# google-research/rigl

Measured on AMD Instinct MI355X. Metric: images/sec/node, ResNet-50 80% ERK RigL step, higher is better.
Workload: dtype bf16

## Files before the change

### rigl_amd/csrc/conv.hip

```cpp
#include <stdlib.h>

#include "common.hpp"

#if defined(RIGL_ABLATE) && RIGL_ABLATE == 1
#define RIGL_MFMA_OR_ABLATE(i, j) acc[i][j][0] += (float)af[i][0] + (float)bfr[j][0];
#else
#define RIGL_MFMA_OR_ABLATE(i, j) acc[i][j] = __builtin_amdgcn_mfma_f32_32x32x16_bf16(bfr[j], af[i], acc[i][j], 0, 0, 0);
#endif

namespace rigl {
namespace k1 {

typedef __attribute__((ext_vector_type(8))) __bf16 bf16x8;
typedef __attribute__((ext_vector_type(2))) __bf16 bf16x2;
typedef __attribute__((ext_vector_type(2))) float f32x2;
typedef __attribute__((ext_vector_type(16))) float f32x16;

constexpr int THREADS = 256;

__device__ __forceinline__ uint16_t f2bf(float f) {
  uint32_t u = __float_as_uint(f);
  if ((u & 0x7FFFFFFFu) > 0x7F800000u) return (uint16_t)((u >> 16) | 0x40u);
  u += 0x7FFFu + ((u >> 16) & 1u);
  return (uint16_t)(u >> 16);
// ... 1089 lines not shown
  return pl;
}

template <int MODE, bool F32>
static void launch_igemm(const IgemmArgs& a0, hipStream_t st) {
  IgemmArgs a = a0;
  const IgemmPlan pl = plan_igemm<MODE>(a);
  if (!F32 && pl.big) {
    RIGL_K_LAUNCH((k_igemm_big<MODE, false>), dim3(pl.grid), dim3(512), (igemm_smem_bytes<2, 2, 32, MODE, false, false, 3, 4>()), st, a);
    return;
  }
  if (pl.cls) launch_igemm_t<MODE, F32, true>(a, dim3(pl.grid), pl.wide_n, pl.dma, st);
  else launch_igemm_t<MODE, F32, false>(a, dim3(pl.grid), pl.wide_n, pl.dma, st);
}

static int check_desc(const RiglConvDesc* d, const char* who) {
  if (!d) return fail(RIGL_EINVAL, "%s: NULL descriptor", who);
  if (d->n <= 0 || d->h <= 0 || d->w <= 0 || d->cin <= 0 || d->ho <= 0 || d->wo <= 0 || d->cout <= 0 || d->kh <= 0 ||
      d->kw <= 0 || d->stride_h <= 0 || d->stride_w <= 0 || d->pad_top < 0 || d->pad_left < 0)
    return fail(RIGL_EINVAL, "%s: non-positive dimension in descriptor", who);
  if ((d->ho - 1) * d->stride_h - d->pad_top >= d->h || (d->wo - 1) * d->stride_w - d->pad_left >= d->w)
    return fail(RIGL_EINVAL, "%s: output size inconsistent with input/stride/pad", who);
  const int64_t lim = (int64_t(1) << 30) - 1;
  if ((int64_t)d->n * d->h * d->w * d->cin > lim || (int64_t)d->n * d->ho * d->wo * d->cout > lim ||
      (int64_t)d->kh * d->kw * d->cin * d->cout > lim)
    return fail(RIGL_EUNSUPPORTED, "%s: tensor exceeds 2^30 elements", who);
  return RIGL_OK;
}

static inline bool small_cin(const RiglConvDesc* d) { return (d->cin % 8) != 0 && d->cin > 4; }
static inline int kpad(const RiglConvDesc* d) { return (d->kh * d->kw * d->cin + 31) / 32 * 32; }

#include "convpp.hpp"
#include "bwd1x1.hpp"
#include "stem.hpp"
#include "c3x3.hpp"
#include "rowstream.hpp"
#include "bwdslice.hpp"

static size_t pp_ksplit_workspace(const RiglConvDesc* d) {
  if (d->cin <= 4 || (d->cin % 8) || (d->cout % 8)) return 0;
  IgemmArgs a = {};
  a.M = d->n * d->ho * d->wo; a.N = d->cout; a.Cred = d->cin; a.a_pix_stride = d->cin; a.KH = d->kh; a.KW = d->kw;
  a.RH = d->ho; a.RW = d->wo; a.GH = d->h; a.GW = d->w; a.sh = d->stride_h; a.sw = d->stride_w;
  const PPPlan p = plan_pp<0>(a);
  if (!pp_ksplit_ok(a, p)) return 0;
  return (size_t)p.grid * 2 * p.bm * p.bn * 4 + align_up((size_t)p.grid * 4, 256);
}

struct WgradPlan { int tm, tn, tiles_ci, tiles_co, splits; int64_t slab; };
static int wgrad_stages(int tm, int tn) { return (tm == 2 && tn == 2) ? 3 : 4; }
static int num_cus() {
  static const int n = [] {
    int dev = 0, v = 0;
    if (hipGetDevice(&dev) != hipSuccess || hipDeviceGetAttribute(&v, hipDeviceAttributeMultiprocessorCount, dev) != hipSuccess || v <= 0) v = 256;
    return v;
  }();
  return n;
}
static WgradPlan plan_wgrad(int M, int cin, int cout, int taps, bool fused = false) {
  WgradPlan p;
  p.tm = cin > 64 ? 2 : 1;
  p.tn = cout > 64 ? 2 : 1;
  p.tiles_ci = (cin + 64 * p.tm - 1) / (64 * p.tm);
  p.tiles_co = (cout + 64 * p.tn - 1) / (64 * p.tn);
  const int64_t base = (int64_t)p.tiles_ci * p.tiles_co * taps;
  const int kt = (M + 63) / 64;
  const int target = 0;
  const int lds = wgrad_stages(p.tm, p.tn) * 32 * 64 * (p.tm + p.tn) * 2;
  const int lds_cu = 160 * 1024;
  int occ = lds_cu / lds;
  if (occ > 4) occ = 4;
  int64_t slots = target > 0 ? target : (int64_t)num_cus() * occ;
  static const int fused_pct = [] { const char* e = getenv("RIGL_WGRAD_FUSED_PCT"); return e ? atoi(e) : 60; }();
  static const int fused_pct_small = [] { const char* e = getenv("RIGL_WGRAD_FUSED_PCT_SMALL"); return e ? atoi(e) : 75; }();
  if (fused && target <= 0) slots = slots * ((p.tm == 2 && p.tn == 2) ? fused_pct : fused_pct_small) / 100;
  int64_t s = slots / base;
  if (s > kt / 4) s = kt / 4;
  if (s < 1) s = 1;
  if (s > 1024) s = 1024;
  p.splits = (int)s;
  p.slab = (int64_t)taps * cin * cout;
  return p;
}

static WgradPlan tiny_wgrad_plan(int M, int cred, int cout, int kh) { return plan_wgrad(M, kh * cred, cout, 1); }

}
}

extern "C" {

size_t rigl_conv2d_workspace_bytes(const RiglConvDesc* d, int32_t which) {
  using namespace rigl;
  using namespace rigl::k1;
  if (!d) return 0;
  const int64_t M = (int64_t)d->n * d->ho * d->wo;
  if (tiny_cin(d)) {
    const TinyGeom tg = tiny_geom(d);
    const size_t xp = align_up((size_t)d->n * tg.hp * tg.wp * 4 * 2, 256);
    if (which == 0) return xp + align_up((size_t)d->cout * d->kh * tg.cred * 2, 256);
    if (which == 2) {
      WgradPlan p = tiny_wgrad_plan((int)M, tg.cred, d->cout, d->kh);
      const size_t generic = xp + align_up((size_t)p.slab * 4, 256) + align_up((size_t)p.splits * p.slab * 4, 256);
      const size_t direct = stem_wgrad_workspace(d);
      return generic > direct ? generic : direct;
    }
    return 0;
  }
  if (small_cin(d)) {
    const int Kp = kpad(d);
    size_t col = align_up((size_t)M * Kp * 2, 256);
    if (which == 0) return col + align_up((size_t)d->cout * Kp * 2, 256);
    if (which == 2) {
      WgradPlan p = plan_wgrad((int)M, Kp, d->cout, 1);
      return col + align_up((size_t)p.splits * p.slab * 4, 256);
    }
    return 0;
  }
  if (which == 0) return pp_ksplit_workspace(d);
  if (which == 2) {
    WgradPlan p = plan_wgrad((int)M, d->cin, d->cout, d->kh * d->kw);
    size_t need = p.splits > 1 ? align_up((size_t)p.splits * p.slab * 4, 256) : 0;
    const size_t npp = align_up(pp_wgrad_workspace(d), 256);
    if (npp > need) need = npp;
    const size_t n11 = align_up(bwd1x1_workspace(d), 256);
    if (n11 > need) need = n11;
    const size_t n33 = align_up(c3x3_wgrad_workspace(d), 256);
    if (n33 > need) need = n33;
    const size_t nbs = align_up(bs_workspace(d), 256);
    if (nbs > need) need = nbs;
    return need;
  }
  return 0;
}

int32_t rigl_conv2d_stats_parts(const RiglConvDesc* d) {
  if (!d || d->cout <= 0 || (d->cout % 8)) return 0;
  const int64_t M = (int64_t)d->n * d->ho * d->wo;
  using namespace rigl::k1;
  if (c3x3_use(d)) return c3x3_stats_parts(d);
  { RsPlan rp; if (rs_use<0>(d, &rp)) return rp.gprime; }
  return (int32_t)((M + 127) / 128);
}

int rigl_masked_conv2d_fwd_stats(const RiglConvDesc* d, const rigl_bf16* x, const rigl_bf16* w_ohwi, rigl_bf16* y,
                                 float* stats, size_t stats_floats, void* workspace, size_t workspace_bytes,
                                 rigl_stream_t stream) {
  using namespace rigl;
  using namespace rigl::k1;
  int rc = check_desc(d, "rigl_masked_conv2d_fwd");
  if (rc) return rc;
  if (!x || !w_ohwi || !y) return fail(RIGL_EINVAL, "rigl_masked_conv2d_fwd: NULL tensor");
  if (d->cout % 8) return fail(RIGL_EUNSUPPORTED, "rigl_masked_conv2d_fwd: cout %% 8 != 0 (use the reference kernel)");
  if (stats && stats_floats < (size_t)rigl_conv2d_stats_parts(d) * 2 * d->cout)
    return fail(RIGL_EWORKSPACE, "rigl_masked_conv2d_fwd_stats: stats buffer %zu floats < %zu", stats_floats,
                (size_t)rigl_conv2d_stats_parts(d) * 2 * d->cout);
  hipStream_t st = as_stream(stream);
  prof_set_tag(d);
  ProfFamily prof(PROF_CONV_FWD);
  IgemmArgs a = {};
  a.C = y; a.M = d->n * d->ho * d->wo; a.N = d->cout; a.ldc = d->cout; a.STATS = stats;
  const size_t need = rigl_conv2d_workspace_bytes(d, 0);
  if ((tiny_cin(d) || small_cin(d)) && need && (!workspace || workspace_bytes < need))
    return fail(RIGL_EWORKSPACE, "rigl_masked_conv2d_fwd: workspace %zu < %zu", workspace_bytes, need);
  if (tiny_cin(d)) {
// ... 563 lines not shown
```

### rigl_amd/csrc/convpp.hpp

```cpp
#pragma once

template <int WM, int WN, int TM, int TN, int PH>
struct PPGeom {
  static_assert(PH == 2 || PH == 1, "phases per K-tile");
  static constexpr int NST = PH == 1 ? 3 : 2;
  static_assert(WM * WN == 8, "eight waves");
  static_assert(TM % 2 == 0 && TN % 2 == 0, "a wave tile splits into 2 x 2 quadrants");
  static constexpr int BM = WM * TM * 32, BN = WN * TN * 32;
  static constexpr int AH_ROWS = BM / 2, BH_ROWS = BN / 2;
  static constexpr int AH_BYTES = AH_ROWS * 128, BH_BYTES = BH_ROWS * 128;
  static constexpr int STAGE = 2 * AH_BYTES + 2 * BH_BYTES;
  static constexpr int NA = AH_ROWS / 64, NB = BH_ROWS / 64;
  static_assert(AH_ROWS % 64 == 0 && BH_ROWS % 64 == 0, "a piece is whole rounds of 8 waves x 8 rows");
  static constexpr int QM = TM / 2, QN = TN / 2;
  static constexpr int EPI_ROWB = TN * 64 + 16;
  static constexpr int EPI_WAVE = QM * 32 * EPI_ROWB;
  static constexpr int EPI_STATS = 8 * EPI_WAVE;
  static constexpr int EPI_ALL = EPI_STATS + 8 * 2 * TN * 32 * 4;
  static constexpr int SMEM = (NST * STAGE > EPI_ALL) ? NST * STAGE : EPI_ALL;
  static_assert(SMEM <= 160 * 1024, "LDS per CU");
};

#define PP_BARRIER()                                                                                     \
  {                                                                                                      \
// ... 242 lines not shown
          const f32x16& a = acc[h * QM + i][j];
          const f32x2 lo = {a[4 * q], a[4 * q + 1]}, hi2 = {a[4 * q + 2], a[4 * q + 3]};
          uint2 pk;
          pk.x = __builtin_bit_cast(uint32_t, __builtin_convertvector(lo, bf16x2));
          pk.y = __builtin_bit_cast(uint32_t, __builtin_convertvector(hi2, bf16x2));
          *reinterpret_cast<uint2*>(stg + row * ROWB + col * 2) = pk;
        }
    const int mrow0 = m0 + wm * TM * 32 + h * QM * 32;
    int mout[ITERS];
#pragma unroll
    for (int it = 0; it < ITERS; ++it) {
      const int lm = mrow0 + it * RPI + rsub;
      if (CLS) {
        int n, rh, rw;
        const int mm = lm < c_cnt ? lm : 0;
        PP_ROW_PIXEL(mm, n, rh, rw);
        mout[it] = lm < c_cnt ? (n * P.RH + rh) * P.RW + rw : -1;
      } else {
        mout[it] = lm < P.M ? lm : -1;
      }
    }
    uint4 addv[ITERS];
    if (P.ADD) {
#pragma unroll
      for (int it = 0; it < ITERS; ++it)
        addv[it] = mout[it] >= 0 ? *reinterpret_cast<const uint4*>(P.ADD + (int64_t)mout[it] * P.ldc + ncol) : make_uint4(0u, 0u, 0u, 0u);
    }
#pragma unroll
    for (int it = 0; it < ITERS; ++it) {
      const int row = it * RPI + rsub, m = mout[it];
      uint4 v = *reinterpret_cast<const uint4*>(stg + row * ROWB + ch * 16);
      if (MODE == 0 && P.STATS) {
        const uint32_t vw[4] = {v.x, v.y, v.z, v.w};
#pragma unroll
        for (int c = 0; c < 8; ++c) {
          const float f = __uint_as_float((c & 1) ? (vw[c >> 1] & 0xFFFF0000u) : (vw[c >> 1] << 16));
          sy[c] += f; sq[c] = fmaf(f, f, sq[c]);
        }
      }
      if (m >= 0) {
        if (P.ADD) {
          const uint4 q = addv[it];
          v.x = add_bf16x2(v.x, q.x); v.y = add_bf16x2(v.y, q.y); v.z = add_bf16x2(v.z, q.z); v.w = add_bf16x2(v.w, q.w);
        }
        store16(C + (int64_t)m * P.ldc + ncol, v);
      }
    }
  }
  if (MODE == 0 && P.STATS) {
#pragma unroll
    for (int off = 8; off < 64; off <<= 1)
#pragma unroll
      for (int c = 0; c < 8; ++c) { sy[c] += __shfl_xor(sy[c], off); sq[c] += __shfl_xor(sq[c], off); }
    float* const wst = reinterpret_cast<float*>(smem + G::EPI_STATS);
    if (lane < 8) {
#pragma unroll
      for (int c = 0; c < 8; ++c) { wst[(wave * 2 + 0) * WCOLS + lane * 8 + c] = sy[c]; wst[(wave * 2 + 1) * WCOLS + lane * 8 + c] = sq[c]; }
    }
    __syncthreads();
    constexpr int WPU = 128 / (TM * 32) > 0 ? 128 / (TM * 32) : 1;
    constexpr int UNITS = BM / 128;
    static_assert(TM * 32 <= 128, "a wave's rows fit one statistics unit");
    for (int idx = tid; idx < UNITS * 2 * BN; idx += 512) {
      const int u = idx / (2 * BN), k = (idx / BN) & 1, col = idx % BN;
      const int wcol = col / WCOLS, cc = col % WCOLS;
      float s = 0.f;
#pragma unroll
      for (int w = 0; w < WPU; ++w) s += wst[(((u * WPU + w) * WN + wcol) * 2 + k) * WCOLS + cc];
      const int64_t unit = (int64_t)tile_m * UNITS + u;
      if (unit * 128 < P.M) P.STATS[unit * 2 * P.N + (int64_t)k * P.N + n0 + col] = s;
    }
  }
}

#undef PP_ROW_PIXEL
template <int WM, int WN, int TM, int TN, int PH, int MODE, bool CLS = false>
__global__ __launch_bounds__(512) void k_igemm_pp(IgemmArgs P) {
  extern __shared__ __attribute__((aligned(1024))) unsigned char smem_pp[];
  pp_igemm_body<WM, WN, TM, TN, PH, MODE, CLS>(P, smem_pp, blockIdx.x, gridDim.x);
}

struct PPWCursor { int kt; int pa[2], pb[2]; };

template <int PH>
__device__ __forceinline__ void pp_wgrad_body(const WgradArgs& P, unsigned char* const smem, uint32_t bid, uint32_t nblk) {
  constexpr int WN = 4, TM = 4, TN = 2;
  using G = PPGeom<2, 4, 4, 2, PH>;
  constexpr int NA = G::NA, NB = G::NB, QM = G::QM, QN = G::QN;
  constexpr int STAGE = G::STAGE, AH_BYTES = G::AH_BYTES, BH_BYTES = G::BH_BYTES;
  static_assert(NA == 2 && NB == 2 && QM == 2 && QN == 1, "256 x 256 tile, 64-pixel K-tiles");

  const int tid = threadIdx.x, lane = tid & 63;
  const int wave = __builtin_amdgcn_readfirstlane(tid >> 6);
  const int wm = wave / WN, wn = wave % WN;
  const int grp = wave >> 2;
  uint32_t b = xcd_remap(bid, nblk);
  const int tco = (int)(b % (uint32_t)P.tiles_co); b /= (uint32_t)P.tiles_co;
  const int tci = (int)(b % (uint32_t)P.tiles_ci); b /= (uint32_t)P.tiles_ci;
  const int taps = P.KH * P.KW;
  const int tap = (int)(b % (uint32_t)taps), split = (int)(b / (uint32_t)taps);
  const int r = tap / P.KW, s = tap - r * P.KW;
  const int ci0 = tci * 256, co0 = tco * 256;
  const int KT_all = (P.M + 63) >> 6;
  const bool il = P.interleave != 0 && P.splits > 1;
  const int kt_begin = il ? split : (int)((int64_t)KT_all * split / P.splits);
  const int kt_step = il ? P.splits : 1;
  const int KT = il ? (split < KT_all ? (KT_all - split + P.splits - 1) / P.splits : 0)
                    : (int)((int64_t)KT_all * (split + 1) / P.splits) - kt_begin;

  const int px_lane = 4 * wave + (lane >> 4);
  const int chunk = (lane & 15) ^ (((lane >> 4) & 3) << 2);
  int chan_a[2], chan_b[2];
#pragma unroll
  for (int h = 0; h < 2; ++h) {
    chan_a[h] = ci0 + (chunk >> 3) * 128 + h * 64 + (chunk & 7) * 8;
    chan_b[h] = co0 + (chunk >> 2) * 64 + h * 32 + (chunk & 3) * 8;
  }
  const __amdgpu_buffer_rsrc_t rsrcA = make_rsrc(P.X, P.x_bytes), rsrcB = make_rsrc(P.DY, P.dy_bytes);
  const int hi0 = r - P.ph, wi0 = s - P.pw;

#define PP_CURSOR_T PPWCursor
#define PP_WCOMPUTE(c_)                                                                                  \
  {                                                                                                      \
    _Pragma("unroll") for (int jj = 0; jj < 2; ++jj) {                                                   \
      const int p_ = ((kt_begin + (c_).kt * kt_step) << 6) + 32 * jj + px_lane;                          \
      const bool ok_ = p_ < P.M;                                                                         \
      const int pp_ = ok_ ? p_ : 0;                                                                      \
      const int t_ = fdiv(pp_, P.fd_wo);                                                                 \
      const int wo_ = pp_ - t_ * P.Wo, n_ = fdiv(t_, P.fd_ho), ho_ = t_ - n_ * P.Ho;                     \
      const int hi_ = ho_ * P.sh + hi0, wi_ = wo_ * P.sw + wi0;                                          \
      const bool oka_ = ok_ && (unsigned)hi_ < (unsigned)P.H && (unsigned)wi_ < (unsigned)P.W;          \
      (c_).pa[jj] = oka_ ? ((n_ * P.H + hi_) * P.W + wi_) * P.x_pix_stride : -1;                         \
      (c_).pb[jj] = ok_ ? p_ * P.Cout : -1;                                                              \
    }                                                                                                    \
  }
#define PP_CURSOR_ZERO(c_) { (c_).kt = 0; PP_WCOMPUTE(c_); }
#define PP_NEXT(c_) { ++(c_).kt; PP_WCOMPUTE(c_); }
#define PP_ISSUE_A(h_, stage_, c_)                                                                       \
  {                                                                                                      \
    _Pragma("unroll") for (int jj = 0; jj < 2; ++jj) {                                                   \
      const int off_ = (c_).pa[jj] >= 0 ? (int)((uint32_t)((c_).pa[jj] + chan_a[h_]) * 2u) : (int)OOB;   \
      __builtin_amdgcn_raw_ptr_buffer_load_lds(                                                          \
          rsrcA, (__attribute__((address_space(3))) void*)(smem + (stage_) * STAGE + (h_) * AH_BYTES + (jj * 8 + wave) * 1024), \
          16, off_, 0, 0, 0);                                                                            \
    }                                                                                                    \
  }
#define PP_ISSUE_B(h_, stage_, c_)                                                                       \
  {                                                                                                      \
    _Pragma("unroll") for (int jj = 0; jj < 2; ++jj) {                                                   \
      const int off_ = (c_).pb[jj] >= 0 ? (int)((uint32_t)((c_).pb[jj] + chan_b[h_]) * 2u) : (int)OOB;   \
      __builtin_amdgcn_raw_ptr_buffer_load_lds(                                                          \
          rsrcB, (__attribute__((address_space(3))) void*)(smem + (stage_) * STAGE + 2 * AH_BYTES + (h_) * BH_BYTES + (jj * 8 + wave) * 1024), \
          16, off_, 0, 0, 0);                                                                            \
    }                                                                                                    \
  }

  const int g = lane >> 4, j16 = lane & 15, rs = (j16 >> 2) & 3;
  const int tr_row = (8 * (g >> 1) + (j16 >> 2)) * 256, tr_low = ((2 * (g & 1) + ((j16 >> 1) & 1)) << 4) + (j16 & 1) * 8;
  int a_tr[QM];
#pragma unroll
  for (int i = 0; i < QM; ++i) a_tr[i] = tr_row + ((((wm * 2 + i) ^ rs) * 4) << 4) + tr_low;
  const int b_tr = tr_row + (((wn ^ rs) * 4) << 4) + tr_low;

  f32x16 acc[TM][TN];
#pragma unroll
  for (int i = 0; i < TM; ++i)
#pragma unroll
    for (int jj = 0; jj < TN; ++jj)
#pragma unroll
      for (int e = 0; e < 16; ++e) acc[i][jj][e] = 0.f;
  constexpr int AF = PH == 1 ? TM : QM;
  bf16x8 af[AF][4], b0[QN][4], b1[QN][4];

#define PP_READ_A(h_, stage_, ab_)                                                                       \
  _Pragma("unroll") for (int i = 0; i < QM; ++i)                                                         \
    _Pragma("unroll") for (int ks = 0; ks < 4; ++ks)                                                     \
      af[(ab_) + i][ks] = lds_read_tr_pair(smem + (stage_) * STAGE + (h_) * AH_BYTES + a_tr[i] + ks * 4096,        \
                                           smem + (stage_) * STAGE + (h_) * AH_BYTES + a_tr[i] + ks * 4096 + 1024);
#define PP_READ_B(dst_, h_, stage_)                                                                      \
  _Pragma("unroll") for (int ks = 0; ks < 4; ++ks)                                                       \
    dst_[0][ks] = lds_read_tr_pair(smem + (stage_) * STAGE + 2 * AH_BYTES + (h_) * BH_BYTES + b_tr + ks * 4096,    \
                                   smem + (stage_) * STAGE + 2 * AH_BYTES + (h_) * BH_BYTES + b_tr + ks * 4096 + 1024);
#define PP_QUAD(ha_, hb_, bsrc_, ab_)                                                                    \
  _Pragma("unroll") for (int ks = 0; ks < 4; ++ks)                                                       \
    _Pragma("unroll") for (int i = 0; i < QM; ++i)                                                       \
      acc[(ha_) * QM + i][(hb_)] = __builtin_amdgcn_mfma_f32_32x32x16_bf16(                              \
          af[(ab_) + i][ks], bsrc_[0][ks], acc[(ha_) * QM + i][(hb_)], 0, 0, 0);
  constexpr int W4 = 2 * NA + 2 * NB, W1 = NA;
#include "convpp_loop.inc"
#undef PP_READ_A
#undef PP_READ_B
#undef PP_QUAD
#undef PP_ISSUE_A
#undef PP_ISSUE_B
#undef PP_NEXT
#undef PP_CURSOR_T
#undef PP_CURSOR_ZERO
#undef PP_WCOMPUTE

  float* const out = P.OUT + (int64_t)split * P.slab_elems + (int64_t)tap * P.Cin * P.Cout;
  constexpr int SROW = 64;
  float* const stg = reinterpret_cast<float*>(smem) + wave * 64 * SROW;
  static_assert(8 * 64 * SROW * 4 <= 2 * STAGE, "epilogue staging fits the K-tile stages");
#pragma unroll
  for (int h = 0; h < 2; ++h) {
#pragma unroll
    for (int i = 0; i < QM; ++i)
#pragma unroll
      for (int jj = 0; jj < TN; ++jj)
#pragma unroll
        for (int e = 0; e < 16; ++e)
          stg[(i * 32 + (e & 3) + 8 * (e >> 2) + 4 * (lane >> 5)) * SROW + jj * 32 + (lane & 31)] = acc[h * QM + i][jj][e];
#pragma unroll
    for (int it = 0; it < 16; ++it) {
      const int row = it * 4 + (lane >> 4), c4 = (lane & 15) * 4;
      const float4 v = *reinterpret_cast<const float4*>(stg + row * SROW + c4);
      const int ci = ci0 + wm * 128 + h * 64 + row, co = co0 + wn * 64 + c4;
      *reinterpret_cast<float4*>(out + (int64_t)ci * P.Cout + co) = v;
    }
  }
}

template <int PH>
__global__ __launch_bounds__(512) void k_wgrad_pp(WgradArgs P) {
  extern __shared__ __attribute__((aligned(1024))) unsigned char smem_pp[];
  pp_wgrad_body<PH>(P, smem_pp, blockIdx.x, gridDim.x);
}

template <int WMD, int WND, int TMD, int TND, int PHD, bool CLSD = false>
__global__ __launch_bounds__(512) void k_bwd_pp(IgemmArgs PD, WgradArgs PW, uint32_t nd, uint32_t nw, uint32_t wgrad_first) {
  extern __shared__ __attribute__((aligned(1024))) unsigned char smem_pp[];
  const uint32_t b = blockIdx.x;
  const bool is_w = wgrad_first ? b < nw : b >= nd;
  if (is_w) {
    pp_wgrad_body<2>(PW, smem_pp, wgrad_first ? b : b - nd, nw);
  } else {
    pp_igemm_body<WMD, WND, TMD, TND, PHD, 1, CLSD>(PD, smem_pp, wgrad_first ? b - nw : b, nd);
  }
}

enum { PP_NONE = 0, PP_256x256 = 1, PP_128x256 = 2, PP_256x128 = 3, PP_512x128 = 4 };

struct PPPlan { int variant; unsigned grid; int bm, bn; };



template <int WM, int WN, int TM, int TN, int PH, int MODE, bool CLS = false>
static bool pp_ready() {
  static const bool ready = hipFuncSetAttribute(reinterpret_cast<const void*>(&k_igemm_pp<WM, WN, TM, TN, PH, MODE, CLS>),
                                                hipFuncAttributeMaxDynamicSharedMemorySize,
                                                PPGeom<WM, WN, TM, TN, PH>::SMEM) == hipSuccess;
  return ready;
}
template <int WM, int WN, int TM, int TN, int PH, int MODE, bool CLS = false>
static bool pp_launch_one(dim3 grid, const IgemmArgs& a, hipStream_t st) {
  if (!pp_ready<WM, WN, TM, TN, PH, MODE, CLS>()) return false;
  RIGL_K_LAUNCH((k_igemm_pp<WM, WN, TM, TN, PH, MODE, CLS>), grid, dim3(512), (PPGeom<WM, WN, TM, TN, PH>::SMEM), st, a);
  return true;
}
static int pp_fill_classes(IgemmArgs& a, int bm) {
  const int n_img = a.M / (a.RH * a.RW);
  int tiles = 0;
  for (int c = 0; c < 4; ++c) {
    const int ph = c / a.sw, pw = c % a.sw;
    int hc = 0, wc = 0;
    if (ph < a.sh && c < a.sh * a.sw) { hc = (a.RH - ph + a.sh - 1) / a.sh; wc = (a.RW - pw + a.sw - 1) / a.sw; }
    a.cls_hc[c] = hc > 0 ? hc : 1; a.cls_wc[c] = wc > 0 ? wc : 1;
    a.fd_chc[c] = make_fastdiv(a.cls_hc[c]); a.fd_cwc[c] = make_fastdiv(a.cls_wc[c]);
    a.cls_cnt[c] = hc > 0 && wc > 0 ? n_img * hc * wc : 0;
    a.cls_tile_begin[c] = tiles;
    tiles += (a.cls_cnt[c] + bm - 1) / bm;
  }
  a.cls_tile_begin[4] = tiles;
  a.cls_n = 0; a.cls_interleave = 1 << 30;
  for (int c = 0; c < 4; ++c) {
    const int tc = a.cls_tile_begin[c + 1] - a.cls_tile_begin[c];
    if (tc > 0) { a.cls_ids[a.cls_n++] = c; if (tc < a.cls_interleave) a.cls_interleave = tc; }
  }
  if (a.cls_n == 0) { a.cls_n = 1; a.cls_ids[0] = 0; a.cls_interleave = 0; }
  return tiles;
}
static inline bool pp_strided(const IgemmArgs& a) { return a.sh > 1 || a.sw > 1; }
template <int MODE>
static int pp_tiles_m(const IgemmArgs& a, int bm) {
  if (MODE == 1 && pp_strided(a)) { IgemmArgs t = a; return pp_fill_classes(t, bm); }
  return (a.M + bm - 1) / bm;
}

static inline void pp_dims(int variant, int& bm, int& bn) {
  switch (variant) {
    case PP_256x256: bm = 256; bn = 256; break;
    case PP_128x256: bm = 128; bn = 256; break;
    case PP_256x128: bm = 256; bn = 128; break;
    case PP_512x128: bm = 512; bn = 128; break;
    default: bm = bn = 0;
  }
}

template <int MODE>
static bool pp_legal(const IgemmArgs& a, int variant) {
  int bm, bn;
  pp_dims(variant, bm, bn);
  if (!bm) return false;
  if (a.Cred % 64 || a.a_pix_stride != a.Cred) return false;
  if (a.N % bn) return false;
  if (a.KH * a.KW > 32) return false;
  if (MODE == 1 && (a.sh > 2 || a.sw > 2)) return false;
  if (a.BNX) return false;
  if (a.M < bm) return false;
  return true;
}

static int pp_bwd_dgrad_variant(const IgemmArgs& a) {
  const int pp_bwd = RIGL_TUNE("pp_bwd", -1);
  if (pp_bwd == 0) return PP_NONE;
  const int64_t m_out = (int64_t)(a.M / (a.RH * a.RW)) * a.GH * a.GW;
  if (a.N % 256 || a.Cred % 256 || m_out < 256 || a.KH * a.KW > 32 || a.BNX || a.sh > 2 || a.sw > 2) return PP_NONE;
  if (pp_bwd > 0) return pp_bwd == 2 ? PP_128x256 : PP_256x256;
  const int kt_d = ((a.KH + a.sh - 1) / a.sh) * ((a.KW + a.sw - 1) / a.sw) * (a.Cred / 64);
  if (kt_d < RIGL_TUNE("pp_bwd_min_kt", 16)) return PP_NONE;
  const int64_t rows = a.M / (a.sh * a.sw);
  return ((rows + 255) / 256) * (a.N / 256) >= 90 ? PP_256x256 : PP_128x256;
}

template <int MODE>
static PPPlan plan_pp(const IgemmArgs& a) {
  PPPlan p = {PP_NONE, 0u, 0, 0};
  const int forced = MODE == 0 ? RIGL_TUNE("pp_fwd", -1) : RIGL_TUNE("pp_dgrad", -1);
  int v = PP_NONE;
  if (forced >= 0) v = forced;
  else if (MODE == 0) {
    const int kt = a.KH * a.KW * (a.Cred / 64);
    const int64_t fill = (int64_t)num_cus() * 3 / 4;
    if (kt >= 8) {
      if (a.N % 256 == 0) v = (int64_t)((a.M + 255) / 256) * (a.N / 256) >= fill ? PP_256x256 : PP_128x256;
      else if (a.N % 128 == 0) v = (int64_t)((a.M + 511) / 512) * (a.N / 128) >= fill ? PP_512x128 : PP_256x128;
    }
  }
  else v = pp_bwd_dgrad_variant(a);
  if (v == PP_NONE || !pp_legal<MODE>(a, v)) return p;
  pp_dims(v, p.bm, p.bn);
  p.variant = v;
  p.grid = (unsigned)(pp_tiles_m<MODE>(a, p.bm) * (a.N / p.bn));
  return p;
}

static inline bool pp_ksplit_ok(const IgemmArgs& a, const PPPlan& p) {
  if (!p.variant || RIGL_TUNE("pp_ksplit", 1) == 0) return false;
  const int kt = a.KH * a.KW * (a.Cred / 64);
  const int min_kt = a.RH * a.RW <= 64 ? 32 : RIGL_TUNE("pp_ksplit_min_kt", 48);
  return 2 * (int64_t)p.grid <= (int64_t)num_cus() && kt >= min_kt;
}

template <int MODE>
static bool launch_pp(const PPPlan& p, const IgemmArgs& a0, hipStream_t st) {
  IgemmArgs a = a0;
  a.fd_rw = make_fastdiv(a.RW); a.fd_rh = make_fastdiv(a.RH);
  a.tiles_n = a.N / p.bn;
  const dim3 grid(MODE == 0 && a.ksplit == 2 ? 2 * p.grid : p.grid);
  if constexpr (MODE == 1) {
    if (pp_strided(a)) {
      pp_fill_classes(a, p.bm);
      switch (p.variant) {
        case PP_256x256: return pp_launch_one<2, 4, 4, 2, 2, 1, true>(grid, a, st);
        case PP_128x256: return pp_launch_one<2, 4, 2, 2, 1, 1, true>(grid, a, st);
        case PP_256x128: return pp_launch_one<4, 2, 2, 2, 1, 1, true>(grid, a, st);
        case PP_512x128: return pp_launch_one<4, 2, 4, 2, 2, 1, true>(grid, a, st);
        default: return false;
      }
    }
  }
  switch (p.variant) {
    case PP_256x256: return pp_launch_one<2, 4, 4, 2, 2, MODE>(grid, a, st);
    case PP_128x256: return pp_launch_one<2, 4, 2, 2, 1, MODE>(grid, a, st);
    case PP_256x128: return pp_launch_one<4, 2, 2, 2, 1, MODE>(grid, a, st);
    case PP_512x128: return pp_launch_one<4, 2, 4, 2, 2, MODE>(grid, a, st);
    default: return false;
  }
}

struct PPBwdPlan {
  bool use;
  int tiles_ci, tiles_co, splits;
  int64_t slab;
  unsigned nd, nw;
  bool wgrad_first;
};

static inline bool pp_wgrad_legal(const RiglConvDesc* d) {
  const int64_t M = (int64_t)d->n * d->ho * d->wo;
  return d->cin % 256 == 0 && d->cout % 256 == 0 && M >= 256 && d->kh * d->kw <= 32;
}
static inline int pp_wgrad_max_splits(const RiglConvDesc* d) {
  const int64_t M = (int64_t)d->n * d->ho * d->wo, kt_all = (M + 63) / 64;
  const int64_t base = (int64_t)d->kh * d->kw * (d->cin / 256) * (d->cout / 256);
  const int64_t dw_bytes = (int64_t)d->kh * d->kw * d->cin * d->cout * 4;
  int64_t s = kt_all / 4;
  const int64_t by_slots = (2 * (int64_t)num_cus() + base - 1) / base, by_bytes = ((int64_t)RIGL_TUNE("pp_slab_mb", 40) << 20) / dw_bytes;
  if (s > by_slots) s = by_slots;
  if (s > by_bytes) s = by_bytes;
  return (int)(s < 1 ? 1 : s);
}
static inline size_t pp_wgrad_workspace(const RiglConvDesc* d) {
  if (!pp_wgrad_legal(d)) return 0;
  const int sp = pp_wgrad_max_splits(d);
  return sp > 1 ? (size_t)sp * d->kh * d->kw * d->cin * d->cout * 4 : 0;
}

static PPBwdPlan plan_wgrad_pp(const RiglConvDesc* d, unsigned nd, int kt_d) {
  PPBwdPlan p = {};
  p.tiles_ci = d->cin / 256; p.tiles_co = d->cout / 256;
  p.slab = (int64_t)d->kh * d->kw * d->cin * d->cout;
  const int64_t M = (int64_t)d->n * d->ho * d->wo, kt_all = (M + 63) / 64;
  const int64_t base = (int64_t)d->kh * d->kw * p.tiles_ci * p.tiles_co, cus = num_cus();
  const int64_t room = base > cus / 4 ? base : cus / 4;
  const int64_t slots = ((int64_t)nd + room + cus - 1) / cus * cus;
  int64_t s = (slots - (int64_t)nd) / base;
  const int smax = pp_wgrad_max_splits(d);
  if (s > smax) s = smax;
  if (s < 1) s = 1;
  p.splits = (int)s;
  p.nd = nd; p.nw = (unsigned)(base * s);
  p.wgrad_first = kt_all / s >= kt_d;
  p.use = true;
  return p;
}

static WgradArgs pp_wgrad_args(const RiglConvDesc* d, const rigl_bf16* x, const rigl_bf16* dy, const PPBwdPlan& p, float* dw,
                               void* workspace) {
  WgradArgs a = {};
  a.interleave = RIGL_TUNE("wgrad_il", 1);
  a.X = x; a.DY = dy; a.M = d->n * d->ho * d->wo; a.Cin = d->cin; a.Cout = d->cout; a.KH = d->kh; a.KW = d->kw;
  a.H = d->h; a.W = d->w; a.Ho = d->ho; a.Wo = d->wo; a.sh = d->stride_h; a.sw = d->stride_w; a.ph = d->pad_top; a.pw = d->pad_left;
  a.tiles_ci = p.tiles_ci; a.tiles_co = p.tiles_co; a.splits = p.splits; a.slab_elems = p.slab;
  a.x_bytes = (uint32_t)((size_t)d->n * d->h * d->w * d->cin * 2);
  a.dy_bytes = (uint32_t)((size_t)a.M * d->cout * 2);
  a.x_pix_stride = d->cin;
  a.fd_wo = make_fastdiv(d->wo); a.fd_ho = make_fastdiv(d->ho);
  a.OUT = p.splits > 1 ? static_cast<float*>(workspace) : dw;
  return a;
}

static bool pp_wgrad_launch(const PPBwdPlan& p, const WgradArgs& aw, hipStream_t st) {
  static const bool ready = hipFuncSetAttribute(reinterpret_cast<const void*>(&k_wgrad_pp<2>),
                                                hipFuncAttributeMaxDynamicSharedMemorySize,
                                                PPGeom<2, 4, 4, 2, 2>::SMEM) == hipSuccess;
  if (!ready) return false;
  RIGL_K_LAUNCH((k_wgrad_pp<2>), dim3(p.nw), dim3(512), (PPGeom<2, 4, 4, 2, 2>::SMEM), st, aw);
  return true;
}
template <int WMD, int WND, int TMD, int TND, int PHD, bool CLSD>
static bool pp_bwd_launch_one(const IgemmArgs& ad, const WgradArgs& aw, unsigned nd, unsigned nw, bool wgrad_first, hipStream_t st) {
  constexpr int SM_D = PPGeom<WMD, WND, TMD, TND, PHD>::SMEM, SM_W = PPGeom<2, 4, 4, 2, 2>::SMEM, SM = SM_D > SM_W ? SM_D : SM_W;
  static const bool ready = hipFuncSetAttribute(reinterpret_cast<const void*>(&k_bwd_pp<WMD, WND, TMD, TND, PHD, CLSD>),
                                                hipFuncAttributeMaxDynamicSharedMemorySize, SM) == hipSuccess;
  if (!ready) return false;
  RIGL_K_LAUNCH((k_bwd_pp<WMD, WND, TMD, TND, PHD, CLSD>), dim3(nd + nw), dim3(512), SM, st, ad, aw, nd, nw, (uint32_t)(wgrad_first ? 1u : 0u));
  return true;
}
static bool pp_bwd_launch(int dvar, bool strided, const IgemmArgs& ad, const WgradArgs& aw, const PPBwdPlan& pw, hipStream_t st) {
  if (strided) {
    switch (dvar) {
      case PP_256x256: return pp_bwd_launch_one<2, 4, 4, 2, 2, true>(ad, aw, pw.nd, pw.nw, pw.wgrad_first, st);
      case PP_128x256: return pp_bwd_launch_one<2, 4, 2, 2, 1, true>(ad, aw, pw.nd, pw.nw, pw.wgrad_first, st);
      default: return false;
    }
  }
  switch (dvar) {
    case PP_256x256: return pp_bwd_launch_one<2, 4, 4, 2, 2, false>(ad, aw, pw.nd, pw.nw, pw.wgrad_first, st);
    case PP_128x256: return pp_bwd_launch_one<2, 4, 2, 2, 1, false>(ad, aw, pw.nd, pw.nw, pw.wgrad_first, st);
    default: return false;
  }
}
```

Before: 12680.

## Extend fused backward weight-gradient kernel to 128-channel layers with two-tap tiles

Adds a second weight-gradient tile variant (128x128 channels, two filter taps packed into 256 rows, 32-pixel K blocks, contiguous split ranges). The fused dgrad+wgrad backward launch now applies to convolutions whose channel counts are multiples of 128 rather than 256. In ResNet-50 these are the 3x3 convs with 128 channels, which previously took the unfused path. The change adds PP_256x128 and PP_512x128 dgrad pairings, new split planning, and tap-bounds masking. The risks are lower per-tile arithmetic intensity, a larger split workspace, and possible misplanning of the work order.

```diff
diff --git a/rigl_amd/csrc/conv.hip b/rigl_amd/csrc/conv.hip
--- a/rigl_amd/csrc/conv.hip
+++ b/rigl_amd/csrc/conv.hip
@@ -1195,6 +1195,10 @@
   p.splits = (int)s;
   p.slab = (int64_t)taps * cin * cout;
   return p;
+}
+
+static int fused_wgrad_splits(const RiglConvDesc* d) {
+  return plan_wgrad(d->n * d->ho * d->wo, d->cin, d->cout, d->kh * d->kw, true).splits;
 }
 
 static WgradPlan tiny_wgrad_plan(int M, int cred, int cout, int kh) { return plan_wgrad(M, kh * cred, cout, 1); }
diff --git a/rigl_amd/csrc/convpp.hpp b/rigl_amd/csrc/convpp.hpp
--- a/rigl_amd/csrc/convpp.hpp
+++ b/rigl_amd/csrc/convpp.hpp
@@ -348,13 +348,19 @@
 
 struct PPWCursor { int kt; int pa[2], pb[2]; };
 
-template <int PH>
+template <int WT> struct PPWTile;
+template <> struct PPWTile<0> { static constexpr int WM = 2, WN = 4, TM = 4, TN = 2, BCI = 256, BCO = 256, TAPS = 1; };
+template <> struct PPWTile<1> { static constexpr int WM = 4, WN = 2, TM = 2, TN = 2, BCI = 128, BCO = 128, TAPS = 2; };
+
+template <int WT, int PH>
 __device__ __forceinline__ void pp_wgrad_body(const WgradArgs& P, unsigned char* const smem, uint32_t bid, uint32_t nblk) {
-  constexpr int WN = 4, TM = 4, TN = 2;
-  using G = PPGeom<2, 4, 4, 2, PH>;
+  using T = PPWTile<WT>;
+  constexpr int WM = T::WM, WN = T::WN, TM = T::TM, TN = T::TN;
+  using G = PPGeom<WM, WN, TM, TN, PH>;
   constexpr int NA = G::NA, NB = G::NB, QM = G::QM, QN = G::QN;
   constexpr int STAGE = G::STAGE, AH_BYTES = G::AH_BYTES, BH_BYTES = G::BH_BYTES;
-  static_assert(NA == 2 && NB == 2 && QM == 2 && QN == 1, "256 x 256 tile, 64-pixel K-tiles");
+  static_assert(NA == 2 && QN == 1 && TN == 2 && WM * TM == 8, "256-row tiles of 64-pixel K-tiles, two column halves");
+  static_assert(WT == 0 ? (NB == 2 && QM == 2) : (NB == 1 && QM == 1 && PH == 1), "tile geometry");
 
   const int tid = threadIdx.x, lane = tid & 63;
   const int wave = __builtin_amdgcn_readfirstlane(tid >> 6);
@@ -363,39 +369,44 @@
   uint32_t b = xcd_remap(bid, nblk);
   const int tco = (int)(b % (uint32_t)P.tiles_co); b /= (uint32_t)P.tiles_co;
   const int tci = (int)(b % (uint32_t)P.tiles_ci); b /= (uint32_t)P.tiles_ci;
-  const int taps = P.KH * P.KW;
-  const int tap = (int)(b % (uint32_t)taps), split = (int)(b / (uint32_t)taps);
-  const int r = tap / P.KW, s = tap - r * P.KW;
-  const int ci0 = tci * 256, co0 = tco * 256;
-  const int KT_all = (P.M + 63) >> 6;
-  const bool il = P.interleave != 0 && P.splits > 1;
+  const int taps = P.KH * P.KW, tslots = (taps + T::TAPS - 1) / T::TAPS;
+  const int tslot = (int)(b % (uint32_t)tslots), split = (int)(b / (uint32_t)tslots);
+  const int ci0 = tci * T::BCI, co0 = tco * T::BCO;
+  const int KT_all = WT == 0 ? (P.M + 63) >> 6 : (P.M + 31) >> 5;
+  const bool il = WT == 0 && P.interleave != 0 && P.splits > 1;
   const int kt_begin = il ? split : (int)((int64_t)KT_all * split / P.splits);
+  const int kt_end = (int)((int64_t)KT_all * (split + 1) / P.splits);
   const int kt_step = il ? P.splits : 1;
   const int KT = il ? (split < KT_all ? (KT_all - split + P.splits - 1) / P.splits : 0)
-                    : (int)((int64_t)KT_all * (split + 1) / P.splits) - kt_begin;
+                    : WT == 0 ? kt_end - kt_begin : (kt_end - kt_begin + 1) >> 1;
 
   const int px_lane = 4 * wave + (lane >> 4);
   const int chunk = (lane & 15) ^ (((lane >> 4) & 3) << 2);
+  const int arow = (chunk >> 2) / QM * TM * 32 + (chunk >> 2) % QM * 32 + (chunk & 3) * 8;
+  const int a_tap = T::TAPS == 1 ? tslot : tslot * 2 + (arow >> 7);
+  const bool a_tap_ok = a_tap < taps;
   int chan_a[2], chan_b[2];
 #pragma unroll
   for (int h = 0; h < 2; ++h) {
-    chan_a[h] = ci0 + (chunk >> 3) * 128 + h * 64 + (chunk & 7) * 8;
-    chan_b[h] = co0 + (chunk >> 2) * 64 + h * 32 + (chunk & 3) * 8;
+    chan_a[h] = ci0 + ((arow + h * QM * 32) & (T::BCI - 1));
+    chan_b[h] = WT == 0 ? co0 + (chunk >> 2) * 64 + h * 32 + (chunk & 3) * 8 : co0 + chunk * 8;
   }
   const __amdgpu_buffer_rsrc_t rsrcA = make_rsrc(P.X, P.x_bytes), rsrcB = make_rsrc(P.DY, P.dy_bytes);
-  const int hi0 = r - P.ph, wi0 = s - P.pw;
+  const int a_r = a_tap_ok ? a_tap / P.KW : 0, a_s = a_tap_ok ? a_tap - a_r * P.KW : 0;
+  const int hi0 = a_r - P.ph, wi0 = a_s - P.pw;
 
 #define PP_CURSOR_T PPWCursor
 #define PP_WCOMPUTE(c_)                                                                                  \
   {                                                                                                      \
     _Pragma("unroll") for (int jj = 0; jj < 2; ++jj) {                                                   \
-      const int p_ = ((kt_begin + (c_).kt * kt_step) << 6) + 32 * jj + px_lane;                          \
-      const bool ok_ = p_ < P.M;                                                                         \
+      const int blk_ = WT == 0 ? 2 * (kt_begin + (c_).kt * kt_step) + jj : kt_begin + 2 * (c_).kt + jj;   \
+      const int p_ = blk_ * 32 + px_lane;                                                                \
+      const bool ok_ = (WT == 0 || blk_ < kt_end) && p_ < P.M;                                           \
       const int pp_ = ok_ ? p_ : 0;                                                                      \
       const int t_ = fdiv(pp_, P.fd_wo);                                                                 \
       const int wo_ = pp_ - t_ * P.Wo, n_ = fdiv(t_, P.fd_ho), ho_ = t_ - n_ * P.Ho;                     \
       const int hi_ = ho_ * P.sh + hi0, wi_ = wo_ * P.sw + wi0;                                          \
-      const bool oka_ = ok_ && (unsigned)hi_ < (unsigned)P.H && (unsigned)wi_ < (unsigned)P.W;          \
+      const bool oka_ = ok_ && a_tap_ok && (unsigned)hi_ < (unsigned)P.H && (unsigned)wi_ < (unsigned)P.W; \
       (c_).pa[jj] = oka_ ? ((n_ * P.H + hi_) * P.W + wi_) * P.x_pix_stride : -1;                         \
       (c_).pb[jj] = ok_ ? p_ * P.Cout : -1;                                                              \
     }                                                                                                    \
@@ -413,10 +424,12 @@
   }
 #define PP_ISSUE_B(h_, stage_, c_)                                                                       \
   {                                                                                                      \
-    _Pragma("unroll") for (int jj = 0; jj < 2; ++jj) {                                                   \
-      const int off_ = (c_).pb[jj] >= 0 ? (int)((uint32_t)((c_).pb[jj] + chan_b[h_]) * 2u) : (int)OOB;   \
+    _Pragma("unroll") for (int jj = 0; jj < NB; ++jj) {                                                  \
+      const int q_ = WT == 0 ? jj : (h_);                                                                \
+      const int ch_ = WT == 0 ? chan_b[h_] : chan_b[0];                                                  \
+      const int off_ = (c_).pb[q_] >= 0 ? (int)((uint32_t)((c_).pb[q_] + ch_) * 2u) : (int)OOB;          \
       __builtin_amdgcn_raw_ptr_buffer_load_lds(                                                          \
-          rsrcB, (__attribute__((address_space(3))) void*)(smem + (stage_) * STAGE + 2 * AH_BYTES + (h_) * BH_BYTES + (jj * 8 + wave) * 1024), \
+          rsrcB, (__attribute__((address_space(3))) void*)(smem + (stage_) * STAGE + 2 * AH_BYTES + (WT == 0 ? (h_) * BH_BYTES : 0) + (q_ * 8 + wave) * 1024), \
           16, off_, 0, 0, 0);                                                                            \
     }                                                                                                    \
   }
@@ -425,8 +438,11 @@
   const int tr_row = (8 * (g >> 1) + (j16 >> 2)) * 256, tr_low = ((2 * (g & 1) + ((j16 >> 1) & 1)) << 4) + (j16 & 1) * 8;
   int a_tr[QM];
 #pragma unroll
-  for (int i = 0; i < QM; ++i) a_tr[i] = tr_row + ((((wm * 2 + i) ^ rs) * 4) << 4) + tr_low;
-  const int b_tr = tr_row + (((wn ^ rs) * 4) << 4) + tr_low;
+  for (int i = 0; i < QM; ++i) a_tr[i] = tr_row + ((((wm * QM + i) ^ rs) * 4) << 4) + tr_low;
+  int b_tr[2];
+#pragma unroll
+  for (int h = 0; h < 2; ++h)
+    b_tr[h] = WT == 0 ? h * BH_BYTES + tr_row + (((wn ^ rs) * 4) << 4) + tr_low : tr_row + ((((wn * 2 + h) ^ rs) * 4) << 4) + tr_low;
 
   f32x16 acc[TM][TN];
 #pragma unroll
@@ -445,8 +461,8 @@
                                            smem + (stage_) * STAGE + (h_) * AH_BYTES + a_tr[i] + ks * 4096 + 1024);
 #define PP_READ_B(dst_, h_, stage_)                                                                      \
   _Pragma("unroll") for (int ks = 0; ks < 4; ++ks)                                                       \
-    dst_[0][ks] = lds_read_tr_pair(smem + (stage_) * STAGE + 2 * AH_BYTES + (h_) * BH_BYTES + b_tr + ks * 4096,    \
-                                   smem + (stage_) * STAGE + 2 * AH_BYTES + (h_) * BH_BYTES + b_tr + ks * 4096 + 1024);
+    dst_[0][ks] = lds_read_tr_pair(smem + (stage_) * STAGE + 2 * AH_BYTES + b_tr[h_] + ks * 4096,        \
+                                   smem + (stage_) * STAGE + 2 * AH_BYTES + b_tr[h_] + ks * 4096 + 1024);
 #define PP_QUAD(ha_, hb_, bsrc_, ab_)                                                                    \
   _Pragma("unroll") for (int ks = 0; ks < 4; ++ks)                                                       \
     _Pragma("unroll") for (int i = 0; i < QM; ++i)                                                       \
@@ -464,10 +480,10 @@
 #undef PP_CURSOR_ZERO
 #undef PP_WCOMPUTE
 
-  float* const out = P.OUT + (int64_t)split * P.slab_elems + (int64_t)tap * P.Cin * P.Cout;
+  float* const out = P.OUT + (int64_t)split * P.slab_elems;
   constexpr int SROW = 64;
-  float* const stg = reinterpret_cast<float*>(smem) + wave * 64 * SROW;
-  static_assert(8 * 64 * SROW * 4 <= 2 * STAGE, "epilogue staging fits the K-tile stages");
+  float* const stg = reinterpret_cast<float*>(smem) + wave * QM * 32 * SROW;
+  static_assert(8 * QM * 32 * SROW * 4 <= 2 * STAGE, "epilogue staging fits the K-tile stages");
 #pragma unroll
   for (int h = 0; h < 2; ++h) {
 #pragma unroll
@@ -477,29 +493,34 @@
 #pragma unroll
         for (int e = 0; e < 16; ++e)
           stg[(i * 32 + (e & 3) + 8 * (e >> 2) + 4 * (lane >> 5)) * SROW + jj * 32 + (lane & 31)] = acc[h * QM + i][jj][e];
-#pragma unroll
-    for (int it = 0; it < 16; ++it) {
-      const int row = it * 4 + (lane >> 4), c4 = (lane & 15) * 4;
-      const float4 v = *reinterpret_cast<const float4*>(stg + row * SROW + c4);
-      const int ci = ci0 + wm * 128 + h * 64 + row, co = co0 + wn * 64 + c4;
-      *reinterpret_cast<float4*>(out + (int64_t)ci * P.Cout + co) = v;
-    }
-  }
-}
-
-template <int PH>
+    const int trow0 = wm * TM * 32 + h * QM * 32;
+    const int tap = T::TAPS == 1 ? tslot : tslot * 2 + (trow0 >> 7);
+    if (tap < taps) {
+      float* const out_t = out + (int64_t)tap * P.Cin * P.Cout;
+#pragma unroll
+      for (int it = 0; it < QM * 8; ++it) {
+        const int row = it * 4 + (lane >> 4), c4 = (lane & 15) * 4;
+        const float4 v = *reinterpret_cast<const float4*>(stg + row * SROW + c4);
+        const int ci = ci0 + ((trow0 + row) & (T::BCI - 1)), co = co0 + wn * 64 + c4;
+        *reinterpret_cast<float4*>(out_t + (int64_t)ci * P.Cout + co) = v;
+      }
+    }
+  }
+}
+
+template <int WT, int PH>
 __global__ __launch_bounds__(512) void k_wgrad_pp(WgradArgs P) {
   extern __shared__ __attribute__((aligned(1024))) unsigned char smem_pp[];
-  pp_wgrad_body<PH>(P, smem_pp, blockIdx.x, gridDim.x);
-}
-
-template <int WMD, int WND, int TMD, int TND, int PHD, bool CLSD = false>
+  pp_wgrad_body<WT, PH>(P, smem_pp, blockIdx.x, gridDim.x);
+}
+
+template <int WMD, int WND, int TMD, int TND, int PHD, bool CLSD = false, int WT = 0>
 __global__ __launch_bounds__(512) void k_bwd_pp(IgemmArgs PD, WgradArgs PW, uint32_t nd, uint32_t nw, uint32_t wgrad_first) {
   extern __shared__ __attribute__((aligned(1024))) unsigned char smem_pp[];
   const uint32_t b = blockIdx.x;
   const bool is_w = wgrad_first ? b < nw : b >= nd;
   if (is_w) {
-    pp_wgrad_body<2>(PW, smem_pp, wgrad_first ? b : b - nd, nw);
+    pp_wgrad_body<WT, WT == 0 ? 2 : 1>(PW, smem_pp, wgrad_first ? b : b - nd, nw);
   } else {
     pp_igemm_body<WMD, WND, TMD, TND, PHD, 1, CLSD>(PD, smem_pp, wgrad_first ? b - nw : b, nd);
   }
@@ -581,11 +602,18 @@
   const int pp_bwd = RIGL_TUNE("pp_bwd", -1);
   if (pp_bwd == 0) return PP_NONE;
   const int64_t m_out = (int64_t)(a.M / (a.RH * a.RW)) * a.GH * a.GW;
-  if (a.N % 256 || a.Cred % 256 || m_out < 256 || a.KH * a.KW > 32 || a.BNX || a.sh > 2 || a.sw > 2) return PP_NONE;
-  if (pp_bwd > 0) return pp_bwd == 2 ? PP_128x256 : PP_256x256;
+  if (m_out < 256 || a.KH * a.KW > 32 || a.BNX || a.sh > 2 || a.sw > 2) return PP_NONE;
+  const bool w256 = a.N % 256 == 0 && a.Cred % 256 == 0;
+  const bool w128 = !w256 && a.N % 128 == 0 && a.Cred % 128 == 0 && a.KH * a.KW >= 9 && RIGL_TUNE("pp_wgrad128", 1) != 0;
+  if (!w256 && !w128) return PP_NONE;
+  if (pp_bwd > 0) {
+    const int v = pp_bwd <= PP_512x128 ? pp_bwd : PP_256x256;
+    return (w256 ? (v == PP_256x256 || v == PP_128x256) : (v == PP_256x128 || v == PP_512x128)) ? v : PP_NONE;
+  }
   const int kt_d = ((a.KH + a.sh - 1) / a.sh) * ((a.KW + a.sw - 1) / a.sw) * (a.Cred / 64);
   if (kt_d < RIGL_TUNE("pp_bwd_min_kt", 16)) return PP_NONE;
   const int64_t rows = a.M / (a.sh * a.sw);
+  if (w128) return ((rows + 511) / 512) * (a.N / 128) >= 90 ? PP_512x128 : PP_256x128;
   return ((rows + 255) / 256) * (a.N / 256) >= 90 ? PP_256x256 : PP_128x256;
 }
 
@@ -647,19 +675,34 @@
 
 struct PPBwdPlan {
   bool use;
+  int wt;
   int tiles_ci, tiles_co, splits;
   int64_t slab;
   unsigned nd, nw;
   bool wgrad_first;
 };
 
-static inline bool pp_wgrad_legal(const RiglConvDesc* d) {
+static inline int pp_wgrad_tile(const RiglConvDesc* d) {
   const int64_t M = (int64_t)d->n * d->ho * d->wo;
-  return d->cin % 256 == 0 && d->cout % 256 == 0 && M >= 256 && d->kh * d->kw <= 32;
-}
-static inline int pp_wgrad_max_splits(const RiglConvDesc* d) {
+  const int taps = d->kh * d->kw;
+  if (M < 256 || taps > 32) return -1;
+  if (d->cin % 256 == 0 && d->cout % 256 == 0) return 0;
+  if (d->cin % 128 == 0 && d->cout % 128 == 0 && taps >= 9 && RIGL_TUNE("pp_wgrad128", 1) != 0) return 1;
+  return -1;
+}
+static inline bool pp_wgrad_legal(const RiglConvDesc* d) { return pp_wgrad_tile(d) >= 0; }
+static inline int64_t pp_wgrad_base(const RiglConvDesc* d, int wt, int* tiles_ci = nullptr, int* tiles_co = nullptr) {
+  const int bc = wt == 1 ? 128 : 256, taps = d->kh * d->kw;
+  const int tci = d->cin / bc, tco = d->cout / bc;
+  if (tiles_ci) *tiles_ci = tci;
+  if (tiles_co) *tiles_co = tco;
+  return (int64_t)(wt == 1 ? (taps + 1) / 2 : taps) * tci * tco;
+}
+static int fused_wgrad_splits(const RiglConvDesc* d);
+static inline int pp_wgrad_max_splits(const RiglConvDesc* d, int wt) {
+  if (wt == 1) return fused_wgrad_splits(d);
   const int64_t M = (int64_t)d->n * d->ho * d->wo, kt_all = (M + 63) / 64;
-  const int64_t base = (int64_t)d->kh * d->kw * (d->cin / 256) * (d->cout / 256);
+  const int64_t base = pp_wgrad_base(d, wt);
   const int64_t dw_bytes = (int64_t)d->kh * d->kw * d->cin * d->cout * 4;
   int64_t s = kt_all / 4;
   const int64_t by_slots = (2 * (int64_t)num_cus() + base - 1) / base, by_bytes = ((int64_t)RIGL_TUNE("pp_slab_mb", 40) << 20) / dw_bytes;
@@ -668,26 +711,28 @@
   return (int)(s < 1 ? 1 : s);
 }
 static inline size_t pp_wgrad_workspace(const RiglConvDesc* d) {
-  if (!pp_wgrad_legal(d)) return 0;
-  const int sp = pp_wgrad_max_splits(d);
+  const int wt = pp_wgrad_tile(d);
+  if (wt < 0) return 0;
+  const int sp = pp_wgrad_max_splits(d, wt);
   return sp > 1 ? (size_t)sp * d->kh * d->kw * d->cin * d->cout * 4 : 0;
 }
 
 static PPBwdPlan plan_wgrad_pp(const RiglConvDesc* d, unsigned nd, int kt_d) {
   PPBwdPlan p = {};
-  p.tiles_ci = d->cin / 256; p.tiles_co = d->cout / 256;
+  p.wt = pp_wgrad_tile(d);
+  if (p.wt < 0) return p;
   p.slab = (int64_t)d->kh * d->kw * d->cin * d->cout;
   const int64_t M = (int64_t)d->n * d->ho * d->wo, kt_all = (M + 63) / 64;
-  const int64_t base = (int64_t)d->kh * d->kw * p.tiles_ci * p.tiles_co, cus = num_cus();
+  const int64_t base = pp_wgrad_base(d, p.wt, &p.tiles_ci, &p.tiles_co), cus = num_cus();
   const int64_t room = base > cus / 4 ? base : cus / 4;
   const int64_t slots = ((int64_t)nd + room + cus - 1) / cus * cus;
   int64_t s = (slots - (int64_t)nd) / base;
-  const int smax = pp_wgrad_max_splits(d);
-  if (s > smax) s = smax;
+  const int smax = pp_wgrad_max_splits(d, p.wt);
+  if (s > smax || p.wt == 1) s = smax;
   if (s < 1) s = 1;
   p.splits = (int)s;
   p.nd = nd; p.nw = (unsigned)(base * s);
-  p.wgrad_first = kt_all / s >= kt_d;
+  p.wgrad_first = (p.wt == 1 ? kt_all / s / 2 : kt_all / s) >= kt_d;
   p.use = true;
   return p;
 }
@@ -707,34 +752,55 @@
   return a;
 }
 
+template <int WT>
+using PPWGeom = PPGeom<PPWTile<WT>::WM, PPWTile<WT>::WN, PPWTile<WT>::TM, PPWTile<WT>::TN, WT == 0 ? 2 : 1>;
+template <int WT>
+static bool pp_wgrad_launch_one(const PPBwdPlan& p, const WgradArgs& aw, hipStream_t st) {
+  constexpr int PH = WT == 0 ? 2 : 1;
+  static const bool ready = hipFuncSetAttribute(reinterpret_cast<const void*>(&k_wgrad_pp<WT, PH>),
+                                                hipFuncAttributeMaxDynamicSharedMemorySize, PPWGeom<WT>::SMEM) == hipSuccess;
+  if (!ready) return false;
+  RIGL_K_LAUNCH((k_wgrad_pp<WT, PH>), dim3(p.nw), dim3(512), (PPWGeom<WT>::SMEM), st, aw);
+  return true;
+}
 static bool pp_wgrad_launch(const PPBwdPlan& p, const WgradArgs& aw, hipStream_t st) {
-  static const bool ready = hipFuncSetAttribute(reinterpret_cast<const void*>(&k_wgrad_pp<2>),
-                                                hipFuncAttributeMaxDynamicSharedMemorySize,
-                                                PPGeom<2, 4, 4, 2, 2>::SMEM) == hipSuccess;
-  if (!ready) return false;
-  RIGL_K_LAUNCH((k_wgrad_pp<2>), dim3(p.nw), dim3(512), (PPGeom<2, 4, 4, 2, 2>::SMEM), st, aw);
-  return true;
-}
-template <int WMD, int WND, int TMD, int TND, int PHD, bool CLSD>
+  return p.wt == 1 ? pp_wgrad_launch_one<1>(p, aw, st) : pp_wgrad_launch_one<0>(p, aw, st);
+}
+template <int WMD, int WND, int TMD, int TND, int PHD, bool CLSD, int WT>
 static bool pp_bwd_launch_one(const IgemmArgs& ad, const WgradArgs& aw, unsigned nd, unsigned nw, bool wgrad_first, hipStream_t st) {
-  constexpr int SM_D = PPGeom<WMD, WND, TMD, TND, PHD>::SMEM, SM_W = PPGeom<2, 4, 4, 2, 2>::SMEM, SM = SM_D > SM_W ? SM_D : SM_W;
-  static const bool ready = hipFuncSetAttribute(reinterpret_cast<const void*>(&k_bwd_pp<WMD, WND, TMD, TND, PHD, CLSD>),
+  constexpr int SM_D = PPGeom<WMD, WND, TMD, TND, PHD>::SMEM, SM_W = PPWGeom<WT>::SMEM, SM = SM_D > SM_W ? SM_D : SM_W;
+  static const bool ready = hipFuncSetAttribute(reinterpret_cast<const void*>(&k_bwd_pp<WMD, WND, TMD, TND, PHD, CLSD, WT>),
                                                 hipFuncAttributeMaxDynamicSharedMemorySize, SM) == hipSuccess;
   if (!ready) return false;
-  RIGL_K_LAUNCH((k_bwd_pp<WMD, WND, TMD, TND, PHD, CLSD>), dim3(nd + nw), dim3(512), SM, st, ad, aw, nd, nw, (uint32_t)(wgrad_first ? 1u : 0u));
+  RIGL_K_LAUNCH((k_bwd_pp<WMD, WND, TMD, TND, PHD, CLSD, WT>), dim3(nd + nw), dim3(512), SM, st, ad, aw, nd, nw, (uint32_t)(wgrad_first ? 1u : 0u));
   return true;
 }
 static bool pp_bwd_launch(int dvar, bool strided, const IgemmArgs& ad, const WgradArgs& aw, const PPBwdPlan& pw, hipStream_t st) {
+  if (pw.wt == 1) {
+    if (strided) {
+      switch (dvar) {
+        case PP_256x128: return pp_bwd_launch_one<4, 2, 2, 2, 1, true, 1>(ad, aw, pw.nd, pw.nw, pw.wgrad_first, st);
+        case PP_512x128: return pp_bwd_launch_one<4, 2, 4, 2, 2, true, 1>(ad, aw, pw.nd, pw.nw, pw.wgrad_first, st);
+        default: return false;
+      }
+    }
+    switch (dvar) {
+      case PP_256x128: return pp_bwd_launch_one<4, 2, 2, 2, 1, false, 1>(ad, aw, pw.nd, pw.nw, pw.wgrad_first, st);
+      case PP_512x128: return pp_bwd_launch_one<4, 2, 4, 2, 2, false, 1>(ad, aw, pw.nd, pw.nw, pw.wgrad_first, st);
+      default: return false;
+    }
+  }
+  if (pw.wt != 0) return false;
   if (strided) {
     switch (dvar) {
-      case PP_256x256: return pp_bwd_launch_one<2, 4, 4, 2, 2, true>(ad, aw, pw.nd, pw.nw, pw.wgrad_first, st);
-      case PP_128x256: return pp_bwd_launch_one<2, 4, 2, 2, 1, true>(ad, aw, pw.nd, pw.nw, pw.wgrad_first, st);
+      case PP_256x256: return pp_bwd_launch_one<2, 4, 4, 2, 2, true, 0>(ad, aw, pw.nd, pw.nw, pw.wgrad_first, st);
+      case PP_128x256: return pp_bwd_launch_one<2, 4, 2, 2, 1, true, 0>(ad, aw, pw.nd, pw.nw, pw.wgrad_first, st);
       default: return false;
     }
   }
   switch (dvar) {
-    case PP_256x256: return pp_bwd_launch_one<2, 4, 4, 2, 2, false>(ad, aw, pw.nd, pw.nw, pw.wgrad_first, st);
-    case PP_128x256: return pp_bwd_launch_one<2, 4, 2, 2, 1, false>(ad, aw, pw.nd, pw.nw, pw.wgrad_first, st);
+    case PP_256x256: return pp_bwd_launch_one<2, 4, 4, 2, 2, false, 0>(ad, aw, pw.nd, pw.nw, pw.wgrad_first, st);
+    case PP_128x256: return pp_bwd_launch_one<2, 4, 2, 2, 1, false, 0>(ad, aw, pw.nd, pw.nw, pw.wgrad_first, st);
     default: return false;
   }
 }
```

After: 12720 (median of 6 runs). No clear change (+0.4%).
